# Bebra777228/PolGen-RVC

Measured on AMD Instinct MI355X. Metric: real-time-factor (audio-sec/wall-sec) per GPU, 30s@16kHz RMVPE->48kHz, higher is better.
Workload: dtype f32 (conv products as 3 fp16 MFMAs of a hi/lo split, fp32 accumulate; fp32 elsewhere)

## Files before the change

### polgen-rvc_amd/csrc/api.hip

```cpp
#include "api_internal.h"

using namespace rvcx;
using namespace rvcx::api;

bool rvcx::api::localize_overflow(Ctx& c) {
  WeightRegion* best_r = nullptr;
  int best = 0, best_i = -1;
  for (WeightRegion* r : all_regions(c, nullptr)) {
    int i = -1;
    const int v = r->first_overflow(&i);
    if (v > best) {
      best = v;
      best_i = i;
      best_r = r;
    }
  }
  if (!best_r) return false;
  best_r->drop_flag(best_i);
  return true;
}

void rvcx::api::reset_after_failure(Ctx& c) {
  (void)hipDeviceSynchronize();
  c.arena.reset();
// ... 292 lines not shown

int rvcx_weights_clone(rvcx_ctx* ctx, rvcx_ctx* src) {
  CtxLock ga, gb;
  if (ctx && src && ctx != src) {
    ga = CtxLock(ctx->mu, std::defer_lock);
    gb = CtxLock(src->mu, std::defer_lock);
    std::lock(ga, gb);
  }
  API_BEGIN_ONCE(ctx)
  if (!src) fail("weights_clone: null source context");
  if (src->c.device != C->device) fail("weights_clone: contexts live on different devices (use the RCCL broadcast)");
  uint64_t ha = 0, hb = 0;
  std::vector<WeightRegion*> ra = all_regions(src->c, &ha), rb = all_regions(*C, &hb);
  if (ha != hb || ra.size() != rb.size()) fail("weights_clone: the two contexts hold different model layouts");
  RVCX_HIP(hipDeviceSynchronize());
  for (size_t r = 0; r < ra.size(); ++r) {
    if (ra[r]->n_chunks() != rb[r]->n_chunks()) fail("weights_clone: chunk lists differ");
    for (int i = 0; i < ra[r]->n_chunks(); ++i) {
      if (ra[r]->chunk_used(i) != rb[r]->chunk_used(i)) fail("weights_clone: chunk sizes differ");
      RVCX_HIP(hipMemcpy(rb[r]->chunk_base(i), ra[r]->chunk_base(i), ra[r]->chunk_used(i), hipMemcpyDeviceToDevice));
    }
    rb[r]->adopt();
  }
  API_END
}

int rvcx_weights_adopt(rvcx_ctx* ctx) {
  API_BEGIN_ONCE(ctx)
  RVCX_HIP(hipDeviceSynchronize());
  for (WeightRegion* r : all_regions(*C, nullptr)) r->adopt();
  API_END
}

int rvcx_load_rmvpe(rvcx_ctx* ctx, const rvcx_rmvpe_cfg* cfg, const rvcx_tensor* tbl, int n) {
  API_BEGIN_ONCE(ctx)
  TensorTable t = make_table(tbl, n);
  C->rmvpe = rmvpe_load(*C, *cfg, t);
  (void)bigru_probe_publish();
  API_END
}

int rvcx_load_crepe(rvcx_ctx* ctx, const rvcx_tensor* tbl, int n) {
  API_BEGIN_ONCE(ctx)
  TensorTable t = make_table(tbl, n);
  C->crepe = crepe_load(*C, t);
  API_END
}

int rvcx_load_fcpe(rvcx_ctx* ctx, const rvcx_fcpe_cfg* cfg, const rvcx_tensor* tbl, int n) {
  API_BEGIN_ONCE(ctx)
  TensorTable t = make_table(tbl, n);
  C->fcpe = fcpe_load(*C, *cfg, t);
  API_END
// ... 76 lines not shown
```

### polgen-rvc_amd/csrc/conv.h

```cpp
#pragma once
#include "common.h"

namespace rvcx {

enum Act { ACT_NONE = 0, ACT_LRELU = 1, ACT_RELU = 2, ACT_GELU = 3, ACT_TANH = 4, ACT_SIGMOID = 5 };
enum OutMode { OUT_NORMAL = 0, OUT_SHUF1D = 1, OUT_SHUF2D = 2, OUT_TRANSPOSED = 3 };
enum Acc2 { ACC2_NONE = 0, ACC2_SET = 1, ACC2_ADD = 2, ACC2_ADD_DIV = 3 };

struct ConvArgs {
  const float* x = nullptr;
  const float* w = nullptr;
  const void* w_h3 = nullptr;
  const void* x_split = nullptr;
  void* y_split = nullptr;
  const float* bias = nullptr;
  const float* res = nullptr;
  float* y = nullptr;
  float* y2 = nullptr;
  const int* lens_in = nullptr;
  const int* lens_out = nullptr;
  int B = 1;
  int Cin_g = 0, Cin_gp = 0, Cout_g = 0, Cout_gp = 0, groups = 1;
  int Tin = 0;
  int Nout = 0;
  int ksize = 1, kw = 1, rowpitch = 0, dil = 1, pad = 0, stride = 1;
  long x_bs = 0, y_bs = 0, res_bs = 0, y2_bs = 0;
  int x_cs = 0, y_cs = 0, res_cs = 0, y2_cs = 0;
  int pre_act = ACT_NONE;
  float pre_slope = 0.f;
  int act = ACT_NONE;
  float act_slope = 0.f;
  int out_mode = OUT_NORMAL;
  int sh_s = 1, sh_pad = 0, sh_cout = 0, sh_tout = 0;
  int wp_in = 0, wp_out = 0;
  int zero_wp = 0;
  int acc2_mode = ACC2_NONE;
  float acc2_div = 1.f;
  const float* nz_har = nullptr;
  const float* nz_w = nullptr;
  const float* nz_b = nullptr;
  const int* nz_lens = nullptr;
  int nz_k = 0, nz_stride = 1, nz_pad = 0, nz_wstride = 0;
  long nz_bs = 0;
  int nz_len = 0;
  float* part = nullptr;
  long part_cap = 0;
  long part_cap_item = 0;
  int ci_chunk = 0, kk_chunk = 0, wrow = 0, off_min = 0;
  int splitk = 1;
  long long* trace = nullptr;
  int stagger = 0;
  int stagger_blocks = 0;
  int* ovf = nullptr;
  int* ovf_layer = nullptr;
  int seq = 0;
  int dbg = 0;
};

inline int conv_tap_off(const ConvArgs& a, int kk) {
  return (kk / a.kw) * a.rowpitch + (kk % a.kw) * a.dil - a.pad;
// ... 116 lines not shown
```

### polgen-rvc_amd/csrc/conv.hip

```cpp
#include "conv.h"
#include "conv_device.h"
#include "gemm.h"

#include <algorithm>
#include <cmath>

namespace rvcx {

template <int BM, int BN, int WR, int WC>
__global__ __launch_bounds__(256) void conv_mfma_kernel(const ConvArgs a) {
  constexpr int WM = BM / (32 * WR), WN = BN / (32 * WC);
  static_assert(WR * WC == 4 && WM >= 1 && WN >= 1, "bad tile");
  extern __shared__ float smem[];
  float* As = smem;
  float* Bs = smem + a.kk_chunk * a.ci_chunk * BM;

  const int tid = threadIdx.x, lane = tid & 63, wave = tid >> 6;
  const int wr = wave / WC, wc = wave % WC;
  const int i = lane & 31, h = lane >> 5;
  const int b = blockIdx.z;
  const int mt_per_g = (a.Cout_gp + BM - 1) / BM;
  const int g = blockIdx.y / mt_per_g, mt = blockIdx.y % mt_per_g;
  const int co0 = mt * BM;
  const int n0 = blockIdx.x * BN;
// ... 217 lines not shown
  RVCX_HIP(hipEventRecord(rec.b, stream));
  g_prof.push_back(rec);
}

void conv_launch_gemm(const GemmArgs& a, double flops, hipStream_t stream) {
  if (!g_prof_on) {
    launch_gemm(a, stream);
    return;
  }
  ProfRec rec;
  RVCX_HIP(hipEventCreate(&rec.a));
  RVCX_HIP(hipEventCreate(&rec.b));
  rec.flops = flops;
  rec.cin = a.cin; rec.cout = a.cout; rec.k = 1; rec.nout = (int)a.rows; rec.stride = 1; rec.B = (int)(a.rows / a.T);
  RVCX_HIP(hipEventRecord(rec.a, stream));
  rec.tile = launch_gemm(a, stream);
  RVCX_HIP(hipEventRecord(rec.b, stream));
  g_prof.push_back(rec);
}

void launch_conv(ConvArgs a, hipStream_t stream) {
  RVCX_CHECK(a.Cin_gp % 2 == 0 && a.Cout_gp % 32 == 0, "conv: unpadded weights");
  RVCX_CHECK(a.Nout > 0 && a.B > 0, "conv: empty problem");
  if (g_prof_on) {
    ProfRec rec;
    RVCX_HIP(hipEventCreate(&rec.a));
    RVCX_HIP(hipEventCreate(&rec.b));
    rec.tile = 0;
    rec.flops = conv_flops(a);
    rec.cin = a.Cin_g * a.groups; rec.cout = a.Cout_g * a.groups; rec.k = a.ksize; rec.nout = a.Nout;
    rec.stride = a.stride; rec.B = a.B;
    RVCX_HIP(hipEventRecord(rec.a, stream));
    const int slot = launch_conv_fast(a, stream);
    if (slot >= 0) {
      rec.tile = slot;
      RVCX_HIP(hipEventRecord(rec.b, stream));
      g_prof.push_back(rec);
      return;
    }
    (void)hipEventDestroy(rec.a);
    (void)hipEventDestroy(rec.b);
  } else if (launch_conv_fast(a, stream) >= 0) {
    return;
  }
  int best = -1;
  double best_t = 1e300;
// ... 78 lines not shown
```

### polgen-rvc_amd/csrc/conv_device.h

```cpp
#pragma once
#include "conv.h"

namespace rvcx {

typedef float f32x16 __attribute__((ext_vector_type(16)));

__device__ __forceinline__ void report_h3_overflow(int* ovf, int* layer, int seq) {
  if (ovf) atomicOr(ovf, kErrH3Overflow);
  if (layer) atomicMax(layer, 0x7fffffff - seq);
}

__device__ __forceinline__ float apply_act(float v, int act, float slope) {
  switch (act) {
    case ACT_LRELU: return v > 0.f ? v : v * slope;
    case ACT_RELU: return v > 0.f ? v : 0.f;
    case ACT_GELU: return 0.5f * v * (1.f + erff(v * 0.70710678118654752440f));
    case ACT_TANH: return tanhf(v);
    case ACT_SIGMOID: return 1.f / (1.f + __expf(-v));
    default: return v;
  }
}


__device__ __forceinline__ float noise_conv_at(const ConvArgs& a, int b, int c, int t) {
  const int nz_len = a.nz_lens ? a.nz_lens[b] : a.nz_len;
  const float* hb = a.nz_har + (long)b * a.nz_bs;
  const long p0 = (long)t * a.nz_stride - a.nz_pad;
  float n = 0.f;
  for (int j = 0; j < a.nz_k; ++j) {
    const long p = p0 + j;
    const float hvv = (p >= 0 && p < nz_len) ? hb[p] : 0.f;
    n = fmaf(a.nz_w[(long)j * a.nz_wstride + c], hvv, n);
  }
  return n + (a.nz_b ? a.nz_b[c] : 0.f);
}

__device__ __forceinline__ void store_elem(const ConvArgs& a, int b, int cg, int nn, float v, int len_out) {
  if (a.bias) v += a.bias[cg];
  v = apply_act(v, a.act, a.act_slope);
  if (a.out_mode == OUT_NORMAL) {
    if (a.res) v += a.res[(long)b * a.res_bs + (long)cg * a.res_cs + nn];
    if (nn >= len_out) v = 0.f;
    if (a.zero_wp > 0) {
      const int col = nn % a.zero_wp;
      if (col == 0 || col == a.zero_wp - 1) v = 0.f;
    }
    if (a.y) a.y[(long)b * a.y_bs + (long)cg * a.y_cs + nn] = v;
    if (a.acc2_mode != ACC2_NONE) {
      float* p2 = a.y2 + (long)b * a.y2_bs + (long)cg * a.y2_cs + nn;
      if (a.acc2_mode == ACC2_SET) *p2 = v;
      else if (a.acc2_mode == ACC2_ADD) *p2 = *p2 + v;
      else *p2 = (*p2 + v) / a.acc2_div;
    }
  } else if (a.out_mode == OUT_SHUF1D) {
    const int c = cg / a.sh_s, ph = cg - c * a.sh_s;
    const int t = nn * a.sh_s + ph - a.sh_pad;
    if (t >= 0 && t < a.sh_tout) {
      if (a.res) v += a.res[(long)b * a.res_bs + (long)c * a.res_cs + t];
      if (a.nz_har) v += noise_conv_at(a, b, c, t);
      if (t >= len_out) v = 0.f;
      a.y[(long)b * a.y_bs + (long)c * a.y_cs + t] = v;
// ... 7 lines not shown
      const long rowbase = (long)b * a.y_bs + (long)c * a.y_cs + (long)(2 * irow + pa) * a.wp_out;
      a.y[rowbase + 2 * (jj - 1) + pb + 1] = v;
      if (jj == 1 && pb == 0) a.y[rowbase] = 0.f;
      if (jj == a.wp_in - 2 && pb == 1) a.y[rowbase + a.wp_out - 1] = 0.f;
    }
  } else {
    if (a.res) v += a.res[(long)b * a.res_bs + (long)nn * a.res_cs + cg];
    if (nn >= len_out) v = 0.f;
    a.y[(long)b * a.y_bs + (long)nn * a.y_cs + cg] = v;
  }
}

__device__ __forceinline__ void store_tile(const ConvArgs& a, int b, int g, int co_base, int nn, const f32x16& t,
                                           int len_out) {
  if (nn >= a.Nout) return;
#pragma unroll
  for (int r = 0; r < 16; ++r) {
    const int co = co_base + (r & 3) + 8 * (r >> 2);
    if (co < a.Cout_g) store_elem(a, b, g * a.Cout_g + co, nn, t[r], len_out);
  }
}

__device__ __forceinline__ bool fast_epilogue_ok(const ConvArgs& a) {
  return a.out_mode == OUT_NORMAL && a.act <= ACT_RELU;
}

__device__ __forceinline__ void store_tile_fast(const ConvArgs& a, int b, int co_base, int nn, const f32x16& t,
                                                int len_out) {
  if (nn >= a.Nout) return;
  const float slope = a.act == ACT_NONE ? 1.f : (a.act == ACT_RELU ? 0.f : a.act_slope);
  bool live = nn < len_out;
  if (a.zero_wp > 0) {
    const int col = nn % a.zero_wp;
    live = live && col != 0 && col != a.zero_wp - 1;
  }
  float* yb = a.y ? a.y + (long)b * a.y_bs + nn : nullptr;
  const float* rb = a.res ? a.res + (long)b * a.res_bs + nn : nullptr;
  float* y2b = a.acc2_mode != ACC2_NONE ? a.y2 + (long)b * a.y2_bs + nn : nullptr;
#pragma unroll
  for (int r0 = 0; r0 < 16; r0 += 8) {
    float bv[8], rv[8];
#pragma unroll
    for (int q = 0; q < 8; ++q) {
      const int r = r0 + q;
      const int co = co_base + (r & 3) + 8 * (r >> 2);
      const int cc = co < a.Cout_g ? co : 0;
      bv[q] = a.bias ? a.bias[cc] : 0.f;
// ... 18 lines not shown
          v = live ? v : 0.f;
          if (yb) yb[co * a.y_cs] = v;
          float* p2 = y2b + co * a.y2_cs;
          if (a.acc2_mode == ACC2_SET) *p2 = v;
          else if (a.acc2_mode == ACC2_ADD) *p2 = pv[q] + v;
          else *p2 = (pv[q] + v) / a.acc2_div;
        }
      }
    } else {
#pragma unroll
      for (int q = 0; q < 8; ++q) {
        const int r = r0 + q;
        const int co = co_base + (r & 3) + 8 * (r >> 2);
        if (co < a.Cout_g) {
          float v = t[r] + bv[q];
          v = fmaxf(v, v * slope) + rv[q];
          yb[co * a.y_cs] = live ? v : 0.f;
        }
      }
    }
  }
}

__device__ __forceinline__ void store_tile_shuf1d(const ConvArgs& a, int b, int co_base, int nn, const f32x16& t,
                                                  int len_out) {
  if (nn >= a.Nout) return;
  const int s = a.sh_s;
  float* yb = a.y + (long)b * a.y_bs;
  const float* rb = a.res ? a.res + (long)b * a.res_bs : nullptr;
  const int tbase = nn * s - a.sh_pad;
#pragma unroll
  for (int g = 0; g < 4; ++g) {
    const int cg0 = co_base + 8 * g;
    int c = cg0 / s, ph = cg0 - c * s;
    int cc[4], tt[4];
    bool ok[4];
    float bv[4], rv[4];
#pragma unroll
    for (int q = 0; q < 4; ++q) {
      cc[q] = c;
      tt[q] = tbase + ph;
      ok[q] = cg0 + q < a.Cout_g && tt[q] >= 0 && tt[q] < a.sh_tout;
      bv[q] = (a.bias && cg0 + q < a.Cout_g) ? a.bias[cg0 + q] : 0.f;
      rv[q] = (rb && ok[q]) ? rb[(long)c * a.res_cs + tt[q]] : 0.f;
      if (a.nz_har && ok[q]) rv[q] += noise_conv_at(a, b, c, tt[q]);
      if (++ph == s) {
// ... 17 lines not shown
```

### polgen-rvc_amd/csrc/conv_fast.hip

```cpp
#include <cmath>
#include <cstdlib>

#include "conv.h"
#include "conv_device.h"

#ifdef RVCX_ABLATION
#define RVCX_DBG(a, bit) ((a).dbg & (bit))
#else
#define RVCX_DBG(a, bit) 0
#endif

namespace rvcx {

struct BufRsrc {
#if defined(__HIP_DEVICE_COMPILE__)
  __amdgpu_buffer_rsrc_t r;
#endif
};
constexpr int kBufOob = 0x7ffffff0;
__device__ __forceinline__ BufRsrc make_rsrc(const float* base, int bytes) {
  BufRsrc b;
#if defined(__HIP_DEVICE_COMPILE__)
  b.r = __builtin_amdgcn_make_buffer_rsrc(const_cast<float*>(base), 0, bytes, 0x00020000);
#endif
// ... 222 lines not shown
      tp[5] = wall_clock64();
    }
#endif
  } else if (a.out_mode == OUT_SHUF1D) {
    store_tile_shuf1d(a, b, co_w, nn_w, acc[0][0], len_out);
    if constexpr (WN > 1) store_tile_shuf1d(a, b, co_w, nn_w + 32, acc[0][1], len_out);
    if constexpr (WM > 1) {
      store_tile_shuf1d(a, b, co_w + 32, nn_w, acc[1][0], len_out);
      if constexpr (WN > 1) store_tile_shuf1d(a, b, co_w + 32, nn_w + 32, acc[1][1], len_out);
    }
  } else {
    store_tile(a, b, 0, co_w, nn_w, acc[0][0], len_out);
    if constexpr (WN > 1) store_tile(a, b, 0, co_w, nn_w + 32, acc[0][1], len_out);
    if constexpr (WM > 1) {
      store_tile(a, b, 0, co_w + 32, nn_w, acc[1][0], len_out);
      if constexpr (WN > 1) store_tile(a, b, 0, co_w + 32, nn_w + 32, acc[1][1], len_out);
    }
  }
}

__global__ __launch_bounds__(256) void conv_splitk_finish_kernel(const ConvArgs a) {
  const long per = (long)a.Cout_g * a.Nout, total = per * a.B;
  const int S = a.splitk;
  if ((per & 3) == 0) {
    const long slab = per * a.B;
    for (long idx = (blockIdx.x * 256L + threadIdx.x) * 4; idx < total; idx += (long)gridDim.x * 1024) {
      const int b = idx / per;
      const long r = idx - (long)b * per;
      int co = r / a.Nout, nn = r - (long)co * a.Nout;
      const float* p0 = a.part + (long)b * per + r;
      float v[4] = {0.f, 0.f, 0.f, 0.f};
      for (int s0 = 0; s0 < S; s0 += 8) {
        float4 q[8];
#pragma unroll
        for (int j = 0; j < 8; ++j)
          q[j] = s0 + j < S ? *reinterpret_cast<const float4*>(p0 + (long)(s0 + j) * slab) : make_float4(0.f, 0.f, 0.f, 0.f);
#pragma unroll
        for (int j = 0; j < 8; ++j)
          if (s0 + j < S) {
            v[0] += q[j].x;
            v[1] += q[j].y;
            v[2] += q[j].z;
            v[3] += q[j].w;
          }
      }
      const int len_out = a.lens_out ? a.lens_out[b] : 0x7fffffff;
// ... 171 lines not shown
  p->halo[7] = 300000;
  p->bm[60] = 1;
  p->bn[60] = 1024;
  p->halo[60] = 300001;
  p->bm[kConvtThinSlot] = 128;
  p->bn[kConvtThinSlot] = 32;
  p->halo[kConvtThinSlot] = 300002;
  p->bm[kConv3ThinSlot] = 32;
  p->bn[kConv3ThinSlot] = 30;
  p->halo[kConv3ThinSlot] = 300004;
  p->bm[kConvDeepSlot] = 64;
  p->bn[kConvDeepSlot] = 320;
  p->halo[kConvDeepSlot] = 300003;
  for (int t = 0; t < kNumFast; ++t) {
    const int s = 8 + t;
    p->bm[s] = kFast[t].bm;
    p->bn[s] = kFast[t].bn;
    p->halo[s] = kFast[t].cic == 32 ? 100000 : (kFast[t].halo < 0 ? 200000 : kFast[t].halo * 10);
  }
}

void launch_splitk_finish(const ConvArgs& a, hipStream_t stream) {
  const long total = (long)a.B * a.Cout_g * a.Nout;
  const long work = (((long)a.Cout_g * a.Nout) & 3) == 0 ? cdiv64(total, 4) : total;
  hipLaunchKernelGGL(conv_splitk_finish_kernel, dim3((unsigned)std::min<long>(cdiv64(work, 256), 4096)), dim3(256), 0,
                     stream, a);
}

int launch_conv_fast(ConvArgs& a, hipStream_t stream) {
  if (a.Cin_g == 1 && a.groups == 1 && a.ksize <= kCin1MaxK && a.kw >= 1 && a.ksize % a.kw == 0) {
    hipLaunchKernelGGL(conv_cin1_kernel, dim3(cdiv(a.Nout, 256), cdiv(a.Cout_g, 16), a.B), dim3(256), 0, stream, a);
    RVCX_HIP(hipGetLastError());
    return 7;
  }
  if (convt_thin_ok(a)) {
    launch_convt_thin(a, stream);
    return kConvtThinSlot;
  }
  RVCX_CHECK(!a.nz_har || a.out_mode == OUT_SHUF1D, "conv: a fused noise conv needs a polyphase ConvTranspose1d launch");
  if (conv_cout1_ok(a)) {
    static const bool on = !getenv("RVCX_COUT1") || atoi(getenv("RVCX_COUT1")) != 0;
    if (on) {
      hipLaunchKernelGGL(conv_cout1_kernel<7>, dim3((unsigned)cdiv64(cdiv64(a.Nout, 4), 256), 1, a.B), dim3(256), 0, stream, a);
      RVCX_HIP(hipGetLastError());
      return 60;
    }
  }
// ... 102 lines not shown
```

### polgen-rvc_amd/csrc/conv_h3.hip

```cpp
#include <algorithm>
#include <cmath>
#include <cstdlib>

#include "conv.h"
#include "conv_device.h"
#include "h3_device.h"

#ifdef RVCX_ABLATION
#define H3_DBG(a, bit) ((a).dbg & (bit))
#else
#define H3_DBG(a, bit) 0
#endif

namespace rvcx {

template <int BM, int BN, int WR, int WC, int KKT, int HALO, int STRIDE, bool LIN, bool XS = false>
__global__ __launch_bounds__(256, ((LIN && BM * BN >= 8192) || BN >= 512) ? 2 : 3) void conv_h3_kernel(const ConvArgs a) {
  constexpr int WM = BM / (32 * WR), WN = BN / (32 * WC);
  constexpr int WROW = LIN ? BN : BN * STRIDE + HALO;
  constexpr int NBTILE = LIN ? KKT : 1;
  constexpr int A_ELEMS = KKT * 2 * 2 * BM;
  constexpr int NA = (A_ELEMS + 255) / 256;
  constexpr int B_TASKS = NBTILE * 2 * WROW;
  constexpr int NBT = (B_TASKS + 255) / 256;
// ... 208 lines not shown
    for (int n = 0; n < WN; ++n)
#pragma unroll
      for (int r = 0; r < 16; ++r) acc[m][n][r] *= inv;

  const int co_w = co0 + wr * (WM * 32) + 4 * h, nn_w = n0 + wc * (WN * 32) + i;
  if (H3_DBG(a, 8)) return;
  if (a.splitk > 1) {
    float* pb = a.part + ((long)ks * a.B + b) * a.Cout_g * a.Nout;
#pragma unroll
    for (int m = 0; m < WM; ++m)
#pragma unroll
      for (int n = 0; n < WN; ++n) {
        const int nn = nn_w + n * 32;
        if (nn < a.Nout) {
#pragma unroll
          for (int r = 0; r < 16; ++r) {
            const int co = co_w + m * 32 + (r & 3) + 8 * (r >> 2);
            if (co < a.Cout_g) pb[(long)co * a.Nout + nn] = acc[m][n][r];
          }
        }
      }
    return;
  }
  if (a.y_split) {
    const int c_t = co0 + wr * (WM * 32);
#pragma unroll
    for (int m = 0; m < WM; ++m)
#pragma unroll
      for (int n = 0; n < WN; ++n) store_tile_split(a, b, c_t + m * 32, nn_w + n * 32, h, acc[m][n], len_out);
  } else if (fast_epilogue_ok(a) && a.groups == 1) {
#pragma unroll
    for (int m = 0; m < WM; ++m)
#pragma unroll
      for (int n = 0; n < WN; ++n) store_tile_fast(a, b, co_w + m * 32, nn_w + n * 32, acc[m][n], len_out);
  } else if (a.out_mode == OUT_SHUF1D) {
#pragma unroll
    for (int m = 0; m < WM; ++m)
#pragma unroll
      for (int n = 0; n < WN; ++n) store_tile_shuf1d(a, b, co_w + m * 32, nn_w + n * 32, acc[m][n], len_out);
  } else {
#pragma unroll
    for (int m = 0; m < WM; ++m)
#pragma unroll
      for (int n = 0; n < WN; ++n) store_tile(a, b, grp, co_w + m * 32, nn_w + n * 32, acc[m][n], len_out);
  }
}

// ... 107 lines not shown
        }
      }
    }
    *tile_out = best;
    *s_out = S;
  };
  int best = -1, S = 1;
  select(1, 0, &best, &S);
  static const int tile2_mask = getenv("RVCX_TILE2_MASK") ? atoi(getenv("RVCX_TILE2_MASK")) : 255;
  const int cls = (a.out_mode != OUT_NORMAL) ? 8 : (lin ? 2 : (halo > 64 ? 1 : 4));
  int cls2 = cls;
  if (a.x_split || a.y_split) cls2 |= 16;
  const bool tile_for_batch = (tile2_mask & cls) && (!(cls2 & 16) || (tile2_mask & 16));
  if (best >= 0 && a.B > 1 && tile_for_batch) {
    int b2 = -1, s2 = 1;
    select(a.B, S, &b2, &s2);
    if (b2 >= 0 && s2 == S) best = b2;
  }
  if (best < 0) return -1;
  const H3Cfg& F = kH3[best];
  a.off_min = off_min;
  a.wrow = halo;
  a.splitk = S;
  {
    static int dbg = -1;
    if (dbg < 0) dbg = getenv("RVCX_CONV_DBG") ? atoi(getenv("RVCX_CONV_DBG")) : 0;
    a.dbg = dbg;
  }
  dim3 grid(cdiv(a.Nout, F.bn), cdiv(a.Cout_gp, F.bm), a.B * a.groups * S);
  {
    static const bool log = getenv("RVCX_CONV_LOG") != nullptr;
    if (log)
      fprintf(stderr, "h3 tile %d (%dx%d halo %d) S %d grid %u %u %u B %d Cin %d Cout %d k %d Nout %d xs %d ys %d\n", best,
              F.bm, F.bn, F.halo, S, grid.x, grid.y, grid.z, a.B, a.Cin_g, a.Cout_g, a.ksize, a.Nout, a.x_split != nullptr,
              a.y_split != nullptr);
  }
  hipLaunchKernelGGL(a.x_split ? F.kern_xs : F.kern, grid, dim3(256), 0, stream, a);
  if (S > 1) launch_splitk_finish(a, stream);
  RVCX_HIP(hipGetLastError());
  return h3_slot(best);
}

}
```

### polgen-rvc_amd/csrc/models.h

```cpp
#pragma once
#include <functional>

#include "../../include/rvcx.h"
#include "ctx.h"
#include "layers.h"

namespace rvcx {

struct SynthModel {
  std::shared_ptr<WeightRegion> region = std::make_shared<WeightRegion>();
  rvcx_synth_cfg cfg{};
  int upp = 1;
  int dec_rf_frames = 0;
  ConvW emb_phone;
  const float* emb_pitch = nullptr;
  struct EncLayer {
    ConvW qkv, o, ffn1, ffn2;
    AttFlag att;
    const float *rel_k = nullptr, *rel_v = nullptr;
    const float *g1 = nullptr, *b1 = nullptr, *g2 = nullptr, *b2 = nullptr;
  };
  std::vector<EncLayer> enc;
  ConvW proj;
  struct Flow {
    ConvW pre, post, cond, in_l[3], rs_l[3];
  };
  Flow flows[4];
  ConvW conv_pre, cond, conv_post;
  const float* lin_wb = nullptr;
  struct Stage {
    ConvT1dW up;
    ConvW noise;
    int noise_stride = 1, noise_pad = 0;
    ConvW noise_dense;
    int noise_dense_cin = 0;
    int ch = 0;
    ConvW c1[4][3], c2[4][3];
  };
  std::vector<Stage> stages;
  const float* emb_g = nullptr;
};

std::unique_ptr<SynthModel> synth_load(Ctx& c, const rvcx_synth_cfg& cfg, const TensorTable& t);

struct SynthIO {
  int B = 1, T = 0;
  const int* lens_host = nullptr;
  const float* phone_ct = nullptr;
  const int* pitch = nullptr;
  const float* pitchf = nullptr;
  const int* sid_host = nullptr;
  const float* z_noise = nullptr;
  const float* src_noise = nullptr;
  float* out = nullptr;
  int dec_skip = 0;
  int skip_head = 0;
  float* stats_out = nullptr;
  float* z_out = nullptr;
  hipEvent_t ev_decoder = nullptr;
};
size_t synth_arena_bytes(const SynthModel& m, int B, int T);
void synth_forward(Ctx& c, const SynthModel& m, const SynthIO& io, hipEvent_t* stage_ev );

// ... 141 lines not shown
```

### polgen-rvc_amd/csrc/synth.hip

```cpp
#include <algorithm>
#include <cmath>
#include <cstdlib>

#include "models.h"
#include "ops.h"

namespace rvcx {

std::vector<float> wn_weight(const TensorTable& t, const std::string& p, int dim) {
  if (t.has(p + ".weight")) return t.f32(p + ".weight");
  std::string gn = p + ".parametrizations.weight.original0", vn = p + ".parametrizations.weight.original1";
  if (!t.has(gn)) {
    gn = p + ".weight_g";
    vn = p + ".weight_v";
  }
  std::vector<float> g = t.f32(gn), v = t.f32(vn);
  const auto shp = t.shape(vn);
  RVCX_CHECK(shp.size() == 3, "weight-norm tensor must be 3-D: " + p);
  const int64_t d0 = shp[0], d1 = shp[1], d2 = shp[2];
  std::vector<float> w(v.size());
  if (dim == 0) {
    RVCX_CHECK((int64_t)g.size() == d0, "weight_g shape: " + p);
    for (int64_t a = 0; a < d0; ++a) {
      double ss = 0.0;
// ... 153 lines not shown
    mx = std::max(mx, n);
    sum += n + 1024;
  }
  return (enc + dec + 2 * sum + 9 * mx) * sizeof(float) + ((size_t)64 << 20);
}

namespace {

struct Timer3 {
  Ctx& c;
  hipEvent_t* e;
  Timer3(Ctx& cc, hipEvent_t* ev) : c(cc), e(ev) {}
  void mark(int i) {
    if (e) RVCX_HIP(hipEventRecord(e[i], c.stream));
  }
};

int* upload_ints(Ctx& c, const std::vector<int>& v) {
  int* d = c.arena.alloc<int>(v.size());
  RVCX_HIP(hipMemcpyAsync(d, v.data(), v.size() * sizeof(int), hipMemcpyHostToDevice, c.stream));
  return d;
}

}

void synth_forward(Ctx& c, const SynthModel& m, const SynthIO& io, hipEvent_t* stage_ev) {
  const auto& cf = m.cfg;
  const int B = io.B, T = io.T, hid = cf.hidden_channels, inter = cf.inter_channels, filt = cf.filter_channels;
  const int heads = cf.n_heads, kc = hid / heads, half = inter / 2, gin = cf.gin_channels;
  hipStream_t s = c.stream;
  Arena& A = c.arena;
  Timer3 tm(c, stage_ev);
  tm.mark(0);
  const int head = io.skip_head, Tk = T - head;
  RVCX_CHECK(head >= 0 && Tk > 0, "synth: skip_head outside [0, T)");
  if (head > 0) {
    RVCX_CHECK(io.dec_skip == 0, "synth: dec_skip and skip_head exclude each other");
    if (io.lens_host)
      for (int b = 0; b < B; ++b) RVCX_CHECK(io.lens_host[b] == T, "synth: skip_head needs equal lengths (every item T frames)");
  }

  bool ragged = false;
  if (io.lens_host)
    for (int b = 0; b < B; ++b) ragged |= io.lens_host[b] != T;
  std::vector<const int*> lens_stage(m.stages.size() + 2, nullptr);
  const int* lens = nullptr;
  if (ragged) {
    std::vector<int> l(io.lens_host, io.lens_host + B);
    lens = upload_ints(c, l);
    lens_stage[0] = lens;
    for (size_t i = 0; i < m.stages.size(); ++i) {
      for (auto& x : l) x *= cf.up_rates[i];
      lens_stage[i + 1] = upload_ints(c, l);
    }
  }
  std::vector<int> sidv(io.sid_host, io.sid_host + B);

  const long Tupp = (long)Tk * m.upp;
  const float* pitchf = io.pitchf;
  if (head > 0) {
    float* pf = A.alloc<float>((size_t)B * Tk);
    launch_copy_strided(io.pitchf + head, pf, B, Tk, T, Tk, s);
    pitchf = pf;
  }
  float* har = A.alloc<float>((size_t)B * Tupp);
  std::vector<float*> nz(m.stages.size(), nullptr);
  std::vector<char> nz_fused(m.stages.size(), 0);
  for (size_t i = 0; i < m.stages.size(); ++i) {
    const auto& S = m.stages[i];
    ConvArgs probe = convT1d_args(S.up, nullptr, nullptr, 1, 1, cf.up_rates[i]);
    probe.pre_act = ACT_LRELU;
    probe.pre_slope = 0.1f;
    static const bool fuse_on = !getenv("RVCX_NOISE_FUSE") || atoi(getenv("RVCX_NOISE_FUSE")) != 0;
    static const int fuse_max_k = getenv("RVCX_NOISE_FUSE_K") ? atoi(getenv("RVCX_NOISE_FUSE_K")) : 4;
    nz_fused[i] = fuse_on && S.noise.cin == 1 && S.noise.groups == 1 && S.noise.k >= 1 && S.noise.cout == S.ch &&
                  S.noise.k <= fuse_max_k;
    (void)probe;
  }
  {
// ... 13 lines not shown
      static const bool dense_on = !getenv("RVCX_NOISE_DENSE") || atoi(getenv("RVCX_NOISE_DENSE")) != 0;
      if (dense_on && S.noise_dense_cin > 0 && Tupp == tt * S.noise_stride) {
        const int sp = S.noise_dense_cin, st = S.noise_stride;
        float* x2 = A.alloc<float>((size_t)B * sp * tt);
        RVCX_HIP(hipMemsetAsync(x2, 0, (size_t)B * sp * tt * sizeof(float), sn));
        for (int b = 0; b < B; ++b) launch_transpose(har + (size_t)b * Tupp, x2 + (size_t)b * sp * tt, 1, (int)tt, st, sn);
        ConvArgs a = conv1d_args(S.noise_dense, x2, nz[i], B, (int)tt, (int)tt, 1, 1, 1);
        a.lens_out = lens_stage[i + 1];
        c.conv_on(a, sn);
        continue;
      }
      ConvArgs a = conv1d_args(S.noise, har, nz[i], B, (int)Tupp, (int)tt, S.noise_stride, 1, S.noise_pad);
      a.lens_in = lens_stage[m.stages.size()];
      a.lens_out = lens_stage[i + 1];
      c.conv_on(a, sn);
    }
    if (sn != s) RVCX_HIP(hipEventRecord(c.ev_src[1], sn));
  }

  float* x = A.alloc<float>((size_t)B * hid * T);
  {
    ConvArgs a = conv1d_args(m.emb_phone, io.phone_ct, x, B, T, T);
    a.lens_out = lens;
    c.conv(a);
    launch_embed_pitch(x, m.emb_pitch, io.pitch, B, hid, T, std::sqrt((float)hid), 0.1f, lens, s);
  }
  float* qkv = A.alloc<float>((size_t)B * 3 * hid * T);
  float* att = A.alloc<float>((size_t)B * hid * T);
  float* tmp = A.alloc<float>((size_t)B * hid * T);
  float* hbuf = A.alloc<float>((size_t)B * filt * T);
  float* scratch = A.alloc<float>(attention_scratch_floats(B, heads, T, 10));
  float* asplit = A.alloc<float>(attention_split_floats(B, heads, T));
  const float scale = 1.f / std::sqrt((float)kc);
  for (const auto& L : m.enc) {
    ConvArgs a = conv1d_args(L.qkv, x, qkv, B, T, T);
    a.lens_out = lens;
    c.conv(a);
    launch_attention(qkv, qkv + (size_t)hid * T, qkv + (size_t)2 * hid * T, att, B, heads, kc, T, T,
                     (long)3 * hid * T, (long)hid * T, scale, L.rel_k, L.rel_v, 10, lens, scratch, asplit, s, c.dev_err, L.att.word,
                     ++c.launch_seq, L.att.h3());
    c.flops += attention_flops(B, heads, kc, T);
    a = conv1d_args(L.o, att, tmp, B, T, T);
    a.lens_out = lens;
    conv_set_res(a, x, hid, T);
    c.conv(a);
    launch_layernorm_c(tmp, L.g1, L.b1, x, B, hid, T, 1e-5f, nullptr, s);
    const int k = L.ffn1.k, pl = (k - 1) / 2;
    a = conv1d_args(L.ffn1, x, hbuf, B, T, T, 1, 1, pl);
// ... 4 lines not shown
    a = conv1d_args(L.ffn2, hbuf, tmp, B, T, T, 1, 1, pl);
    a.lens_in = lens;
    a.lens_out = lens;
    conv_set_res(a, x, hid, T);
    c.conv(a);
    launch_layernorm_c(tmp, L.g2, L.b2, x, B, hid, T, 1e-5f, nullptr, s);
  }
  float* stats = io.stats_out ? io.stats_out : A.alloc<float>((size_t)B * 2 * inter * T);
  {
    launch_mask(x, B, hid, T, lens, s);
    ConvArgs a = conv1d_args(m.proj, x, stats, B, T, T);
    a.lens_out = lens;
    c.conv(a);
  }
  tm.mark(1);

  float* z = A.alloc<float>((size_t)B * inter * T);
  float* z2 = A.alloc<float>((size_t)B * inter * T);
  launch_sample_z(stats, io.z_noise, z, B, inter, T, lens, s);
  if (head > 0) {
    launch_copy_strided(z + head, z2, B * inter, Tk, T, Tk, s);
    std::swap(z, z2);
  }
  float* g = A.alloc<float>((size_t)B * gin);
  for (int b = 0; b < B; ++b)
    RVCX_HIP(hipMemcpyAsync(g + (size_t)b * gin, m.emb_g + (size_t)sidv[b] * gin, gin * sizeof(float),
                            hipMemcpyDeviceToDevice, s));
  {
    float* h = att;
    float* xin = qkv;
    float* acts = tmp;
    float* rs = hbuf;
    RVCX_CHECK(filt >= 2 * hid, "buffer reuse assumes filter_channels >= 2*hidden");
    float* wout = A.alloc<float>((size_t)B * hid * T);
    float* mbuf = A.alloc<float>((size_t)B * half * T);
    float* gc = A.alloc<float>((size_t)B * 6 * hid);
    for (int f = 3; f >= 0; --f) {
      const auto& F = m.flows[f];
      launch_flip_channels(z, z2, B, inter, Tk, s);
      std::swap(z, z2);
      ConvArgs a = conv1d_args(F.pre, z, h, B, Tk, Tk);
      a.x_bs = (long)inter * Tk;
      a.lens_out = lens;
      c.conv(a);
      a = conv1d_args(F.cond, g, gc, B, 1, 1);
      c.conv(a);
      for (int i = 0; i < 3; ++i) {
        a = conv1d_args(F.in_l[i], h, xin, B, Tk, Tk, 1, 1, (F.in_l[i].k - 1) / 2);
        a.lens_in = lens;
        a.lens_out = lens;
        c.conv(a);
        launch_wn_gate(xin, gc, i * 2 * hid, 6 * hid, acts, B, hid, Tk, s);
        a = conv1d_args(F.rs_l[i], acts, rs, B, Tk, Tk);
        a.lens_out = lens;
        c.conv(a);
        launch_wn_res_skip(h, wout, rs, B, hid, Tk, i == 2, i == 0, lens, s);
      }
      a = conv1d_args(F.post, wout, mbuf, B, Tk, Tk);
      a.lens_out = lens;
      c.conv(a);
      launch_coupling_sub(z, mbuf, B, half, Tk, lens, s);
    }
  }
  if (io.z_out)
    RVCX_HIP(hipMemcpyAsync(io.z_out, z, (size_t)B * inter * Tk * sizeof(float), hipMemcpyDeviceToDevice, s));
  tm.mark(2);
  if (io.ev_decoder) RVCX_HIP(hipEventRecord(io.ev_decoder, s));

  if (!c.serial) RVCX_HIP(hipStreamWaitEvent(s, c.ev_src[1], 0));
  static const int dec_batch_env = getenv("RVCX_DEC_BATCH") ? std::max(1, atoi(getenv("RVCX_DEC_BATCH"))) : 8;
  bool equal_lens = true;
  if (io.lens_host)
    for (int b = 1; b < B; ++b) equal_lens &= io.lens_host[b] == io.lens_host[0];
  const int dec_batch = equal_lens ? dec_batch_env : 1;
  const int C0 = cf.up_initial_channel;
  const size_t dec_mark = A.mark();
  for (int b0 = 0; b0 < B; b0 += dec_batch) {
    const int db = std::min(dec_batch, B - b0);
    A.reset(dec_mark);
    const bool own = io.lens_host != nullptr && (db == 1 || equal_lens);
    const int Tfull = own ? io.lens_host[b0] - head : Tk;
    RVCX_CHECK(Tfull > 0 && Tfull <= Tk, "synth: item length outside (0, T]");
    const int skip = (io.dec_skip > 0 && (own || !lens) && Tfull - 2 * io.dec_skip > 2 * m.dec_rf_frames) ? io.dec_skip : 0;
    const int Td = Tfull - 2 * skip;
    float* cur = A.alloc<float>((size_t)db * C0 * Td);
    {
      ConvArgs a = conv1d_args(m.conv_pre, z + (size_t)b0 * inter * Tk + skip, cur, db, Td, Td, 1, 1, 3);
      a.x_bs = (long)inter * Tk;
      a.x_cs = Tk;
      a.lens_in = (lens && !own) ? lens + b0 : nullptr;
      c.conv(a);
      float* gcond = A.alloc<float>((size_t)db * C0);
      a = conv1d_args(m.cond, g + (size_t)b0 * gin, gcond, db, 1, 1);
      c.conv(a);
      launch_add_channel_bias(cur, gcond, db, C0, Td, s);
    }
    long Tin = Td, Tin_c = Tk, off = skip;
    for (size_t i = 0; i < m.stages.size(); ++i) {
      const auto& S = m.stages[i];
      const long Tout = Tin * cf.up_rates[i], Tout_c = Tin_c * cf.up_rates[i];
      off *= cf.up_rates[i];
      const size_t n = (size_t)db * S.ch * Tout;
      float* xs = A.alloc<float>(n);
      const size_t stage_mark = A.mark();
      float* xu = A.alloc<float>(n);
      const int nk = cf.n_resblocks;
      float* xcb[4];
      float* xtb[4];
      for (int j = 0; j < nk; ++j) {
        xcb[j] = A.alloc<float>(n);
        xtb[j] = A.alloc<float>(n);
      }
      const int* lin = (lens_stage[i] && !own) ? lens_stage[i] + b0 : nullptr;
      const int* lout = (lens_stage[i + 1] && !own) ? lens_stage[i + 1] + b0 : nullptr;
      ConvArgs a = convT1d_args(S.up, cur, xu, db, (int)Tin, (int)Tout);
      a.pre_act = ACT_LRELU;
      a.pre_slope = 0.1f;
      a.lens_in = lin;
// ... 160 lines not shown
```

Before: 1239.

## Fold flow/embedding elementwise ops into conv epilogues and cache speaker terms

Adds a folded-epilogue mode to the h3 conv kernels so several follow-up elementwise kernels run inside the conv store instead of separately. These are the pitch-embedding add with leaky ReLU, the WaveNet residual/skip update, the coupling subtract, the channel-bias add, and the tanh·sigmoid gate in the split-K finish. It also caches each speaker's conditioning conv outputs (the flow cond and decoder cond) in device memory and drops the cache whenever weights change. The goal is fewer kernel launches and less intermediate memory traffic in the text encoder, flow and decoder-prologue paths. In exchange it adds epilogue branching and more complex store paths, and the cache performs a per-speaker device allocation on first use.

```diff
diff --git a/polgen-rvc_amd/csrc/api.hip b/polgen-rvc_amd/csrc/api.hip
--- a/polgen-rvc_amd/csrc/api.hip
+++ b/polgen-rvc_amd/csrc/api.hip
@@ -338,6 +338,8 @@
     }
     rb[r]->adopt();
   }
+  for (auto& m : C->synths)
+    if (m) m->drop_spk_terms();
   API_END
 }
 
@@ -345,6 +347,8 @@
   API_BEGIN_ONCE(ctx)
   RVCX_HIP(hipDeviceSynchronize());
   for (WeightRegion* r : all_regions(*C, nullptr)) r->adopt();
+  for (auto& m : C->synths)
+    if (m) m->drop_spk_terms();
   API_END
 }
 
diff --git a/polgen-rvc_amd/csrc/conv.h b/polgen-rvc_amd/csrc/conv.h
--- a/polgen-rvc_amd/csrc/conv.h
+++ b/polgen-rvc_amd/csrc/conv.h
@@ -6,6 +6,7 @@
 enum Act { ACT_NONE = 0, ACT_LRELU = 1, ACT_RELU = 2, ACT_GELU = 3, ACT_TANH = 4, ACT_SIGMOID = 5 };
 enum OutMode { OUT_NORMAL = 0, OUT_SHUF1D = 1, OUT_SHUF2D = 2, OUT_TRANSPOSED = 3 };
 enum Acc2 { ACC2_NONE = 0, ACC2_SET = 1, ACC2_ADD = 2, ACC2_ADD_DIV = 3 };
+enum Fold { FOLD_NONE = 0, FOLD_RES_SKIP = 1, FOLD_SUB = 2, FOLD_CBIAS = 3, FOLD_EMBED = 4, FOLD_GATE = 5 };
 
 struct ConvArgs {
   const float* x = nullptr;
@@ -36,6 +37,15 @@
   int zero_wp = 0;
   int acc2_mode = ACC2_NONE;
   float acc2_div = 1.f;
+  int fold = FOLD_NONE;
+  float* f_out = nullptr;
+  const float* f_g = nullptr;
+  const int* f_idx = nullptr;
+  int f_hid = 0, f_first = 0, f_last = 0;
+  float f_scale = 1.f, f_slope = 0.f;
+  int gate_req = 0;
+  int f_gs = 0;
+  bool* f_applied = nullptr;
   const float* nz_har = nullptr;
   const float* nz_w = nullptr;
   const float* nz_b = nullptr;
diff --git a/polgen-rvc_amd/csrc/conv.hip b/polgen-rvc_amd/csrc/conv.hip
--- a/polgen-rvc_amd/csrc/conv.hip
+++ b/polgen-rvc_amd/csrc/conv.hip
@@ -263,6 +263,9 @@
 void launch_conv(ConvArgs a, hipStream_t stream) {
   RVCX_CHECK(a.Cin_gp % 2 == 0 && a.Cout_gp % 32 == 0, "conv: unpadded weights");
   RVCX_CHECK(a.Nout > 0 && a.B > 0, "conv: empty problem");
+  RVCX_CHECK(a.fold == FOLD_NONE || (a.out_mode == OUT_NORMAL && a.act == ACT_NONE && !a.res && a.acc2_mode == ACC2_NONE &&
+                                     !a.y_split && a.groups == 1 && a.zero_wp == 0 && a.y),
+             "conv: a folded epilogue takes a plain 1-D conv (no activation, residual, second output or split store)");
   if (g_prof_on) {
     ProfRec rec;
     RVCX_HIP(hipEventCreate(&rec.a));
diff --git a/polgen-rvc_amd/csrc/conv_device.h b/polgen-rvc_amd/csrc/conv_device.h
--- a/polgen-rvc_amd/csrc/conv_device.h
+++ b/polgen-rvc_amd/csrc/conv_device.h
@@ -35,8 +35,47 @@
   return n + (a.nz_b ? a.nz_b[c] : 0.f);
 }
 
+__device__ __forceinline__ float* fold_dst(const ConvArgs& a, int b, int cg, int nn) {
+  if (a.fold == FOLD_RES_SKIP && (a.f_last || cg >= a.f_hid))
+    return a.f_out + (long)b * a.y_bs + (long)(a.f_last ? cg : cg - a.f_hid) * a.y_cs + nn;
+  return a.y + (long)b * a.y_bs + (long)cg * a.y_cs + nn;
+}
+__device__ __forceinline__ float fold_operand(const ConvArgs& a, int b, int cg, const float* dst, int row) {
+  switch (a.fold) {
+    case FOLD_RES_SKIP: return (a.f_first && (a.f_last || cg >= a.f_hid)) ? 0.f : *dst;
+    case FOLD_SUB: return *dst;
+    case FOLD_CBIAS: return a.f_g[(long)b * a.Cout_g + cg];
+    default: return a.f_g[(long)row * a.Cout_g + cg];
+  }
+}
+__device__ __forceinline__ float fold_value(const ConvArgs& a, int cg, float v, float o, bool live) {
+  const float m = live ? v : 0.f;
+  switch (a.fold) {
+    case FOLD_RES_SKIP:
+      if (!a.f_last && cg < a.f_hid) return live ? o + m : 0.f;
+      if (!a.f_last) return a.f_first ? m : o + m;
+      return live ? (a.f_first ? m : o + m) : 0.f;
+    case FOLD_SUB: return live ? o - m : 0.f;
+    case FOLD_CBIAS: return m + o;
+    default: {
+      float e = (m + o) * a.f_scale;
+      e = e > 0.f ? e : e * a.f_slope;
+      return live ? e : 0.f;
+    }
+  }
+}
+__device__ __forceinline__ void store_elem_fold(const ConvArgs& a, int b, int cg, int nn, float v, bool live) {
+  float* dst = fold_dst(a, b, cg, nn);
+  const int row = a.fold == FOLD_EMBED ? a.f_idx[(long)b * a.Nout + nn] : 0;
+  *dst = fold_value(a, cg, v, fold_operand(a, b, cg, dst, row), live);
+}
+
 __device__ __forceinline__ void store_elem(const ConvArgs& a, int b, int cg, int nn, float v, int len_out) {
   if (a.bias) v += a.bias[cg];
+  if (a.fold != FOLD_NONE) {
+    store_elem_fold(a, b, cg, nn, v, nn < len_out);
+    return;
+  }
   v = apply_act(v, a.act, a.act_slope);
   if (a.out_mode == OUT_NORMAL) {
     if (a.res) v += a.res[(long)b * a.res_bs + (long)cg * a.res_cs + nn];
@@ -90,7 +129,7 @@
 }
 
 __device__ __forceinline__ bool fast_epilogue_ok(const ConvArgs& a) {
-  return a.out_mode == OUT_NORMAL && a.act <= ACT_RELU;
+  return a.out_mode == OUT_NORMAL && a.act <= ACT_RELU && a.fold == FOLD_NONE;
 }
 
 __device__ __forceinline__ void store_tile_fast(const ConvArgs& a, int b, int co_base, int nn, const f32x16& t,
@@ -155,6 +194,33 @@
   }
 }
 
+__device__ __forceinline__ void store_tile_fold(const ConvArgs& a, int b, int co_base, int nn, const f32x16& t,
+                                                int len_out) {
+  if (nn >= a.Nout) return;
+  const bool live = nn < len_out;
+  const int row = a.fold == FOLD_EMBED ? a.f_idx[(long)b * a.Nout + nn] : 0;
+#pragma unroll
+  for (int r0 = 0; r0 < 16; r0 += 8) {
+    float bv[8], ov[8];
+    float* dp[8];
+#pragma unroll
+    for (int q = 0; q < 8; ++q) {
+      const int r = r0 + q;
+      const int co = co_base + (r & 3) + 8 * (r >> 2);
+      const int cc = co < a.Cout_g ? co : 0;
+      bv[q] = a.bias ? a.bias[cc] : 0.f;
+      dp[q] = fold_dst(a, b, cc, nn);
+      ov[q] = fold_operand(a, b, cc, dp[q], row);
+    }
+#pragma unroll
+    for (int q = 0; q < 8; ++q) {
+      const int r = r0 + q;
+      const int co = co_base + (r & 3) + 8 * (r >> 2);
+      if (co < a.Cout_g) *dp[q] = fold_value(a, co, t[r] + bv[q], ov[q], live);
+    }
+  }
+}
+
 __device__ __forceinline__ void store_tile_shuf1d(const ConvArgs& a, int b, int co_base, int nn, const f32x16& t,
                                                   int len_out) {
   if (nn >= a.Nout) return;
diff --git a/polgen-rvc_amd/csrc/conv_fast.hip b/polgen-rvc_amd/csrc/conv_fast.hip
--- a/polgen-rvc_amd/csrc/conv_fast.hip
+++ b/polgen-rvc_amd/csrc/conv_fast.hip
@@ -268,6 +268,41 @@
 __global__ __launch_bounds__(256) void conv_splitk_finish_kernel(const ConvArgs a) {
   const long per = (long)a.Cout_g * a.Nout, total = per * a.B;
   const int S = a.splitk;
+  if (a.fold == FOLD_GATE) {
+    const int H = a.f_hid;
+    const long hper = (long)H * a.Nout, slab = per * a.B;
+    for (long idx = blockIdx.x * 256L + threadIdx.x; idx < hper * a.B; idx += (long)gridDim.x * 256) {
+      const int b = idx / hper;
+      const long r = idx - (long)b * hper;
+      const int c = r / a.Nout;
+      const float* pt = a.part + (long)b * per + r;
+      const float* ps = pt + hper;
+      float vt = 0.f, vs = 0.f;
+      for (int s0 = 0; s0 < S; s0 += 8) {
+        float qt[8], qs[8];
+#pragma unroll
+        for (int j = 0; j < 8; ++j) {
+          qt[j] = s0 + j < S ? pt[(long)(s0 + j) * slab] : 0.f;
+          qs[j] = s0 + j < S ? ps[(long)(s0 + j) * slab] : 0.f;
+        }
+#pragma unroll
+        for (int j = 0; j < 8; ++j)
+          if (s0 + j < S) {
+            vt += qt[j];
+            vs += qs[j];
+          }
+      }
+      if (a.bias) {
+        vt += a.bias[c];
+        vs += a.bias[H + c];
+      }
+      const float* g = a.f_g + (long)b * a.f_gs;
+      const float ta = vt + g[c];
+      const float sa = vs + g[H + c];
+      a.f_out[(long)b * hper + r] = tanhf(ta) * (1.f / (1.f + expf(-sa)));
+    }
+    return;
+  }
   if ((per & 3) == 0) {
     const long slab = per * a.B;
     for (long idx = (blockIdx.x * 256L + threadIdx.x) * 4; idx < total; idx += (long)gridDim.x * 1024) {
@@ -485,7 +520,8 @@
 
 void launch_splitk_finish(const ConvArgs& a, hipStream_t stream) {
   const long total = (long)a.B * a.Cout_g * a.Nout;
-  const long work = (((long)a.Cout_g * a.Nout) & 3) == 0 ? cdiv64(total, 4) : total;
+  const long work = a.fold == FOLD_GATE ? total / 2
+                    : (((long)a.Cout_g * a.Nout) & 3) == 0 ? cdiv64(total, 4) : total;
   hipLaunchKernelGGL(conv_splitk_finish_kernel, dim3((unsigned)std::min<long>(cdiv64(work, 256), 4096)), dim3(256), 0,
                      stream, a);
 }
diff --git a/polgen-rvc_amd/csrc/conv_h3.hip b/polgen-rvc_amd/csrc/conv_h3.hip
--- a/polgen-rvc_amd/csrc/conv_h3.hip
+++ b/polgen-rvc_amd/csrc/conv_h3.hip
@@ -254,7 +254,12 @@
       }
     return;
   }
-  if (a.y_split) {
+  if (a.fold != FOLD_NONE) {
+#pragma unroll
+    for (int m = 0; m < WM; ++m)
+#pragma unroll
+      for (int n = 0; n < WN; ++n) store_tile_fold(a, b, co_w + m * 32, nn_w + n * 32, acc[m][n], len_out);
+  } else if (a.y_split) {
     const int c_t = co0 + wr * (WM * 32);
 #pragma unroll
     for (int m = 0; m < WM; ++m)
@@ -408,6 +413,10 @@
   a.off_min = off_min;
   a.wrow = halo;
   a.splitk = S;
+  if (a.gate_req && S > 1 && a.fold == FOLD_NONE && a.Cout_g == 2 * a.f_hid && !a.lens_out) {
+    a.fold = FOLD_GATE;
+    if (a.f_applied) *a.f_applied = true;
+  }
   {
     static int dbg = -1;
     if (dbg < 0) dbg = getenv("RVCX_CONV_DBG") ? atoi(getenv("RVCX_CONV_DBG")) : 0;
diff --git a/polgen-rvc_amd/csrc/models.h b/polgen-rvc_amd/csrc/models.h
--- a/polgen-rvc_amd/csrc/models.h
+++ b/polgen-rvc_amd/csrc/models.h
@@ -1,5 +1,6 @@
 #pragma once
 #include <functional>
+#include <map>
 
 #include "../../include/rvcx.h"
 #include "ctx.h"
@@ -39,6 +40,20 @@
   };
   std::vector<Stage> stages;
   const float* emb_g = nullptr;
+  struct SpkTerms {
+    float* dev = nullptr;
+    unsigned sig = ~0u;
+  };
+  mutable std::map<int, SpkTerms> spk_terms;
+  void drop_spk_terms() {
+    for (auto& kv : spk_terms)
+      if (kv.second.dev) (void)hipFree(kv.second.dev);
+    spk_terms.clear();
+  }
+  SynthModel() = default;
+  SynthModel(const SynthModel&) = delete;
+  SynthModel& operator=(const SynthModel&) = delete;
+  ~SynthModel() { drop_spk_terms(); }
 };
 
 std::unique_ptr<SynthModel> synth_load(Ctx& c, const rvcx_synth_cfg& cfg, const TensorTable& t);
diff --git a/polgen-rvc_amd/csrc/synth.hip b/polgen-rvc_amd/csrc/synth.hip
--- a/polgen-rvc_amd/csrc/synth.hip
+++ b/polgen-rvc_amd/csrc/synth.hip
@@ -199,6 +199,34 @@
   return d;
 }
 
+bool chain_fold_on() {
+  static const bool on = !getenv("RVCX_CHAIN_FOLD") || atoi(getenv("RVCX_CHAIN_FOLD")) != 0;
+  return on;
+}
+
+constexpr size_t kMaxSpkTerms = 1024;
+
+const float* spk_terms_row(Ctx& c, const SynthModel& m, int sid) {
+  const int hid = m.cfg.hidden_channels, gin = m.cfg.gin_channels, C0 = m.cfg.up_initial_channel;
+  unsigned sig = 0;
+  for (int f = 0; f < 4; ++f) sig |= (conv_h3_ok(m.flows[f].cond) ? 1u : 0u) << f;
+  sig |= (conv_h3_ok(m.cond) ? 1u : 0u) << 4;
+  auto it = m.spk_terms.find(sid);
+  if (it != m.spk_terms.end() && it->second.sig == sig) return it->second.dev;
+  if (it == m.spk_terms.end()) {
+    if (m.spk_terms.size() >= kMaxSpkTerms) return nullptr;
+    SynthModel::SpkTerms e;
+    RVCX_HIP(hipMalloc(&e.dev, ((size_t)4 * 6 * hid + C0) * sizeof(float)));
+    it = m.spk_terms.emplace(sid, e).first;
+  }
+  it->second.sig = sig;
+  float* row = it->second.dev;
+  const float* g = m.emb_g + (size_t)sid * gin;
+  for (int f = 0; f < 4; ++f) c.conv(conv1d_args(m.flows[f].cond, g, row + (size_t)f * 6 * hid, 1, 1, 1));
+  c.conv(conv1d_args(m.cond, g, row + (size_t)4 * 6 * hid, 1, 1, 1));
+  return row;
+}
+
 }
 
 void synth_forward(Ctx& c, const SynthModel& m, const SynthIO& io, hipEvent_t* stage_ev) {
@@ -232,6 +260,8 @@
     }
   }
   std::vector<int> sidv(io.sid_host, io.sid_host + B);
+  const bool chain = chain_fold_on() && conv_h3_enabled();
+  const bool fold = chain && !ragged && head == 0;
 
   const long Tupp = (long)Tk * m.upp;
   const float* pitchf = io.pitchf;
@@ -291,8 +321,17 @@
   {
     ConvArgs a = conv1d_args(m.emb_phone, io.phone_ct, x, B, T, T);
     a.lens_out = lens;
-    c.conv(a);
-    launch_embed_pitch(x, m.emb_pitch, io.pitch, B, hid, T, std::sqrt((float)hid), 0.1f, lens, s);
+    if (fold && conv_h3_ok(m.emb_phone)) {
+      a.fold = FOLD_EMBED;
+      a.f_g = m.emb_pitch;
+      a.f_idx = io.pitch;
+      a.f_scale = std::sqrt((float)hid);
+      a.f_slope = 0.1f;
+      c.conv(a);
+    } else {
+      c.conv(a);
+      launch_embed_pitch(x, m.emb_pitch, io.pitch, B, hid, T, std::sqrt((float)hid), 0.1f, lens, s);
+    }
   }
   float* qkv = A.alloc<float>((size_t)B * 3 * hid * T);
   float* att = A.alloc<float>((size_t)B * hid * T);
@@ -343,10 +382,34 @@
     launch_copy_strided(z + head, z2, B * inter, Tk, T, Tk, s);
     std::swap(z, z2);
   }
-  float* g = A.alloc<float>((size_t)B * gin);
-  for (int b = 0; b < B; ++b)
-    RVCX_HIP(hipMemcpyAsync(g + (size_t)b * gin, m.emb_g + (size_t)sidv[b] * gin, gin * sizeof(float),
-                            hipMemcpyDeviceToDevice, s));
+  const int C0 = cf.up_initial_channel;
+  const size_t flow_terms = (size_t)4 * 6 * hid;
+  const float *gflow = nullptr, *gdec = nullptr;
+  float* g = nullptr;
+  if (chain) {
+    std::vector<const float*> rows(B, nullptr);
+    bool have = true;
+    for (int b = 0; b < B && have; ++b) have = (rows[b] = spk_terms_row(c, m, sidv[b])) != nullptr;
+    if (have && B == 1) {
+      gflow = rows[0];
+      gdec = rows[0] + flow_terms;
+    } else if (have) {
+      float* gf = A.alloc<float>((size_t)B * flow_terms);
+      float* gd = A.alloc<float>((size_t)B * C0);
+      for (int b = 0; b < B; ++b) {
+        RVCX_HIP(hipMemcpyAsync(gf + (size_t)b * flow_terms, rows[b], flow_terms * sizeof(float), hipMemcpyDeviceToDevice, s));
+        RVCX_HIP(hipMemcpyAsync(gd + (size_t)b * C0, rows[b] + flow_terms, C0 * sizeof(float), hipMemcpyDeviceToDevice, s));
+      }
+      gflow = gf;
+      gdec = gd;
+    }
+  }
+  if (!gflow) {
+    g = A.alloc<float>((size_t)B * gin);
+    for (int b = 0; b < B; ++b)
+      RVCX_HIP(hipMemcpyAsync(g + (size_t)b * gin, m.emb_g + (size_t)sidv[b] * gin, gin * sizeof(float),
+                              hipMemcpyDeviceToDevice, s));
+  }
   {
     float* h = att;
     float* xin = qkv;
@@ -364,23 +427,56 @@
       a.x_bs = (long)inter * Tk;
       a.lens_out = lens;
       c.conv(a);
-      a = conv1d_args(F.cond, g, gc, B, 1, 1);
-      c.conv(a);
+      const float* gcf = gflow ? gflow + (size_t)f * 6 * hid : gc;
+      const int gstride = gflow ? (int)flow_terms : 6 * hid;
+      if (!gflow) {
+        a = conv1d_args(F.cond, g, gc, B, 1, 1);
+        c.conv(a);
+      }
       for (int i = 0; i < 3; ++i) {
         a = conv1d_args(F.in_l[i], h, xin, B, Tk, Tk, 1, 1, (F.in_l[i].k - 1) / 2);
         a.lens_in = lens;
         a.lens_out = lens;
+        bool gated = false;
+        if (fold && conv_h3_ok(F.in_l[i])) {
+          a.gate_req = 1;
+          a.f_out = acts;
+          a.f_g = gcf + (size_t)i * 2 * hid;
+          a.f_gs = gstride;
+          a.f_hid = hid;
+          a.f_applied = &gated;
+        }
         c.conv(a);
-        launch_wn_gate(xin, gc, i * 2 * hid, 6 * hid, acts, B, hid, Tk, s);
+        if (!gated) launch_wn_gate(xin, gcf, i * 2 * hid, gstride, acts, B, hid, Tk, s);
         a = conv1d_args(F.rs_l[i], acts, rs, B, Tk, Tk);
         a.lens_out = lens;
-        c.conv(a);
-        launch_wn_res_skip(h, wout, rs, B, hid, Tk, i == 2, i == 0, lens, s);
+        if (fold && conv_h3_ok(F.rs_l[i])) {
+          a.y = h;
+          a.y_bs = (long)hid * Tk;
+          a.y_cs = Tk;
+          a.fold = FOLD_RES_SKIP;
+          a.f_out = wout;
+          a.f_hid = hid;
+          a.f_first = i == 0;
+          a.f_last = i == 2;
+          c.conv(a);
+        } else {
+          c.conv(a);
+          launch_wn_res_skip(h, wout, rs, B, hid, Tk, i == 2, i == 0, lens, s);
+        }
       }
       a = conv1d_args(F.post, wout, mbuf, B, Tk, Tk);
       a.lens_out = lens;
-      c.conv(a);
-      launch_coupling_sub(z, mbuf, B, half, Tk, lens, s);
+      if (fold && conv_h3_ok(F.post)) {
+        a.y = z + (size_t)half * Tk;
+        a.y_bs = (long)inter * Tk;
+        a.y_cs = Tk;
+        a.fold = FOLD_SUB;
+        c.conv(a);
+      } else {
+        c.conv(a);
+        launch_coupling_sub(z, mbuf, B, half, Tk, lens, s);
+      }
     }
   }
   if (io.z_out)
@@ -394,7 +490,6 @@
   if (io.lens_host)
     for (int b = 1; b < B; ++b) equal_lens &= io.lens_host[b] == io.lens_host[0];
   const int dec_batch = equal_lens ? dec_batch_env : 1;
-  const int C0 = cf.up_initial_channel;
   const size_t dec_mark = A.mark();
   for (int b0 = 0; b0 < B; b0 += dec_batch) {
     const int db = std::min(dec_batch, B - b0);
@@ -410,11 +505,21 @@
       a.x_bs = (long)inter * Tk;
       a.x_cs = Tk;
       a.lens_in = (lens && !own) ? lens + b0 : nullptr;
-      c.conv(a);
-      float* gcond = A.alloc<float>((size_t)db * C0);
-      a = conv1d_args(m.cond, g + (size_t)b0 * gin, gcond, db, 1, 1);
-      c.conv(a);
-      launch_add_channel_bias(cur, gcond, db, C0, Td, s);
+      const float* gcond = gdec ? gdec + (size_t)b0 * C0 : nullptr;
+      if (gcond && fold && conv_h3_ok(m.conv_pre)) {
+        a.fold = FOLD_CBIAS;
+        a.f_g = gcond;
+        c.conv(a);
+      } else {
+        c.conv(a);
+        if (!gcond) {
+          float* gc2 = A.alloc<float>((size_t)db * C0);
+          ConvArgs ac = conv1d_args(m.cond, g + (size_t)b0 * gin, gc2, db, 1, 1);
+          c.conv(ac);
+          gcond = gc2;
+        }
+        launch_add_channel_bias(cur, gcond, db, C0, Td, s);
+      }
     }
     long Tin = Td, Tin_c = Tk, off = skip;
     for (size_t i = 0; i < m.stages.size(); ++i) {
```

Result: no change. 1239 (-0.0%).
